# BoxLib-Codes/VARDEN

Hardware: AMD Instinct MI355X
Metric: cells*steps/sec on advance_timestep (higher is better)
Workload: dtype f64; 1 GPU; 3D 256x256x256 single-level variable-density bubble, 1 box(es) of 256^3, MAC+HG projection each step (BASELINE.json configs[1]); parallelism=single GPU, cells=16777216

## Files before the change

### include/varden_amd.h

```cpp
#ifndef VARDEN_AMD_H
#define VARDEN_AMD_H
#include <stddef.h>

#ifdef __cplusplus
extern "C" {
#endif

enum {
  VDN_PERIODIC = -1, VDN_INTERIOR = 0, VDN_INLET = 11, VDN_OUTLET = 12, VDN_SYMMETRY = 13,
  VDN_SLIP_WALL = 14, VDN_NO_SLIP_WALL = 15,
  VDN_REFLECT_ODD = 20, VDN_REFLECT_EVEN = 21, VDN_FOEXTRAP = 22, VDN_EXT_DIR = 23, VDN_HOEXTRAP = 24,
  VDN_BC_PER = -1, VDN_BC_INT = 0, VDN_BC_DIR = 1, VDN_BC_NEU = 2
};

enum { VDN_INITIAL_PROJECTION = 1, VDN_DIVU_ITERS = 2, VDN_PRESSURE_ITERS = 3, VDN_REGULAR_TIMESTEP = 4 };

typedef struct vdn_params {
  int    dm;
  int    nscal;
  int    slope_order;
  int    use_minion;
  int    boussinesq;
  int    stencil_order;
  int    diffusion_type;
// ... 190 lines not shown
        const char *const *names, const vdn_box *pd0, const double *prob_lo, const double *prob_hi,
        double time, const double *dx0, long staging_bytes);
int vdn_fabio_ml_multifab_info (const char *dirname, int *nlev, int *dm, int *ncomp, int nodal[3], int *nboxes, int *rr, double *time);
int vdn_fabio_ml_multifab_boxes(const char *dirname, int lev, vdn_box *boxes, int maxboxes);
int vdn_fabio_ml_multifab_read_d(const char *dirname, int nlev, vdn_multifab *const *mfs, long staging_bytes);
int vdn_checkpoint_write(const char *dirname, int nlev, vdn_multifab *const *state, vdn_multifab *const *pressure,
        const int *rr, double time, double dt, long staging_bytes);
int vdn_checkpoint_info (const char *dirname, int *nlev, double *time, double *dt, int *rr);
int vdn_fabio_ml_multifab_write_plane_d(const char *dirname, int nlev, vdn_multifab *const *mfs, const int *rr,
        const char *const *names, const vdn_box *pd0, const double *prob_lo, const double *prob_hi,
        double time, const double *dx0, long staging_bytes, int ncomp, const int *comps, int nvanish, const int *vanish, double *defect );
int vdn_fabio_ml_multifab_read_plane_d(const char *dirname, int nlev, vdn_multifab *const *mfs, long staging_bytes, int ncomp, const int *comps);
int vdn_checkpoint_write_plane(const char *dirname, int nlev, vdn_multifab *const *state, vdn_multifab *const *pressure,
        const int *rr, double time, double dt, long staging_bytes, int ncomp, const int *comps, int nvanish, const int *vanish, double *defect );
int vdn_make_vorticity_plane(vdn_multifab *vort, int comp, vdn_multifab *u, const double *dx , const vdn_bc_tower *bct);

int  vdn_last_step_timing(double *sec5);
int  vdn_last_solver_stats(int which , int *cycles, double *res0, double *res);
int  vdn_last_bottom_stats(int which , int *calls, int *iters, int *max_iters, int *breakdowns);
int  vdn_last_bottom_form(int which );
int  vdn_last_mac_level_form(void);

int  vdn_k_slope(const vdn_multifab *s, vdn_multifab *slope, int dir, int bccomp, const vdn_bc_tower *bct);
int  vdn_k_velpred(const vdn_multifab *u, vdn_multifab **umac, const vdn_multifab *force,
                   const double *dx, double dt, const vdn_bc_tower *bct);
int  vdn_k_mkflux(const vdn_multifab *s, vdn_multifab **sedge, vdn_multifab **flux,
                  vdn_multifab **umac, const vdn_multifab *force, const vdn_multifab *mac_rhs,
                  const double *dx, double dt, const vdn_bc_tower *bct, int is_vel, const int *is_cons);
int  vdn_k_update(const vdn_multifab *sold, vdn_multifab **umac, vdn_multifab **sedge, vdn_multifab **flux,
                  const vdn_multifab *force, vdn_multifab *snew, const double *dx, double dt,
                  int is_vel, const int *is_cons, const vdn_bc_tower *bct);
int  vdn_k_mkvelforce(vdn_multifab *vel_force, const vdn_multifab *ext_vel_force, const vdn_multifab *s,
                      const vdn_multifab *gp, const vdn_multifab *lapu , double visc_fac,
                      const vdn_bc_tower *bct);
int  vdn_k_mkscalforce(vdn_multifab *scal_force, const vdn_multifab *ext_scal_force,
                       const vdn_multifab *laps , double diff_fac, const vdn_bc_tower *bct);
int  vdn_k_make_at_halftime(vdn_multifab *rhohalf, const vdn_multifab *sold, const vdn_multifab *snew,
                            int in_comp, int out_comp, const vdn_bc_tower *bct);

int  vdn_cc_solve(vdn_multifab *rh, vdn_multifab *phi, vdn_multifab **beta, const double *dx,
                  const int *bc , double rel_eps, double abs_eps, int max_iter,
                  int *cycles, double *res0, double *res);
int  vdn_cc_solve_alpha(vdn_multifab *rh, vdn_multifab *phi, const vdn_multifab *alpha, vdn_multifab **beta, const double *dx,
                        const int *bc , double rel_eps, double abs_eps, int max_iter,
                        int *cycles, double *res0, double *res);
int  vdn_cc_smooth(vdn_multifab *rh, vdn_multifab *phi, vdn_multifab **beta, const double *dx,
// ... 15 lines not shown
```

### varden_amd/advance.py

```python
import ctypes as C

from . import capi
from .boxlib import handle_array
from .capi import check


def _dx(dx):
    flat = [float(v) for lev in dx for v in lev] if hasattr(dx[0], "__len__") else [float(v) for v in dx]
    return (C.c_double * len(flat))(*flat)


def advance_timestep(istep, mla, sold, uold, snew, unew, gp, p, ext_vel_force, ext_scal_force,
                     the_bc_tower, dt, time, dx, press_comp, proj_type):
    lib = capi.load()
    check(lib.vdn_advance_timestep(istep, mla.h, handle_array(sold), handle_array(uold), handle_array(snew),
                                   handle_array(unew), handle_array(gp), handle_array(p),
                                   handle_array(ext_vel_force), handle_array(ext_scal_force), the_bc_tower.h,
                                   float(dt), float(time), _dx(dx), press_comp, proj_type))


def estdt(lev, u, s, gp, ext_vel_force, dx, dtold):
    out = C.c_double()
    check(capi.load().vdn_estdt(lev, u.h, s.h, gp.h, ext_vel_force.h, _dx(dx), float(dtold), C.byref(out)))
    return out.value
# ... 18 lines not shown

def last_solver_stats(which):
    cyc, r0, r = C.c_int(), C.c_double(), C.c_double()
    capi.load().vdn_last_solver_stats(0 if which == "mac" else 1, C.byref(cyc), C.byref(r0), C.byref(r))
    return cyc.value, r0.value, r.value


def last_bottom_stats(which):
    v = [C.c_int() for _ in range(4)]
    check(capi.load().vdn_last_bottom_stats(0 if which == "mac" else 1, *[C.byref(x) for x in v]))
    return dict(calls=v[0].value, iters=v[1].value, max_iters=v[2].value, breakdowns=v[3].value)


def last_bottom_form(which):
    return int(capi.load().vdn_last_bottom_form(0 if which == "mac" else 1))


def _iv(x):
    return (C.c_int * len(x))(*[int(v) for v in x])


def slope(s, slope_mf, dir, bccomp, bct):
    check(capi.load().vdn_k_slope(s.h, slope_mf.h, dir, bccomp, bct.h))


def velpred(u, umac, force, dx, dt, bct):
    check(capi.load().vdn_k_velpred(u.h, handle_array(umac), force.h, _dx(dx), float(dt), bct.h))


def mkflux(s, sedge, flux, umac, force, mac_rhs, dx, dt, bct, is_vel, is_conservative):
    check(capi.load().vdn_k_mkflux(s.h, handle_array(sedge), handle_array(flux), handle_array(umac), force.h, mac_rhs.h,
                                   _dx(dx), float(dt), bct.h, 1 if is_vel else 0, _iv(is_conservative)))


def update(sold, umac, sedge, flux, force, snew, dx, dt, is_vel, is_cons, bct):
    check(capi.load().vdn_k_update(sold.h, handle_array(umac), handle_array(sedge), handle_array(flux), force.h, snew.h,
                                   _dx(dx), float(dt), 1 if is_vel else 0, _iv(is_cons), bct.h))


def mkvelforce(vel_force, ext_vel_force, s, gp, lapu, visc_fac, bct):
    check(capi.load().vdn_k_mkvelforce(vel_force.h, ext_vel_force.h, s.h, gp.h, lapu.h if lapu else None, float(visc_fac), bct.h))


def mkscalforce(scal_force, ext_scal_force, laps, diff_fac, bct):
    check(capi.load().vdn_k_mkscalforce(scal_force.h, ext_scal_force.h, laps.h if laps else None, float(diff_fac), bct.h))

# ... 541 lines not shown
```

### varden_amd/capi.py

```python
import ctypes as C
import os

_HERE = os.path.dirname(os.path.abspath(__file__))
FLAVOUR = "testing" if os.environ.get("VDN_LIB_FLAVOUR") == "testing" else "release"
LIB_PATH = os.path.join(_HERE, "csrc", "libvarden_amd_testing.so" if FLAVOUR == "testing" else "libvarden_amd.so")


class Params(C.Structure):
    _fields_ = [
        ("dm", C.c_int), ("nscal", C.c_int), ("slope_order", C.c_int), ("use_minion", C.c_int),
        ("boussinesq", C.c_int), ("stencil_order", C.c_int), ("diffusion_type", C.c_int),
        ("verbose", C.c_int), ("mg_verbose", C.c_int), ("prob_type", C.c_int),
        ("visc_coef", C.c_double), ("diff_coef", C.c_double), ("cflfac", C.c_double),
        ("max_dt_growth", C.c_double),
        ("u_bc", (C.c_double * 2) * 3), ("v_bc", (C.c_double * 2) * 3), ("w_bc", (C.c_double * 2) * 3),
        ("rho_bc", (C.c_double * 2) * 3), ("trac_bc", (C.c_double * 2) * 3),
        ("mg_nu1", C.c_int), ("mg_nu2", C.c_int), ("mg_nub", C.c_int), ("mg_max_iter", C.c_int),
        ("hg_max_iter", C.c_int), ("hg_nu1", C.c_int), ("hg_nu2", C.c_int), ("hg_nub", C.c_int),
        ("hg_omega", C.c_double), ("mac_rel_eps", C.c_double), ("hg_rel_eps", C.c_double),
        ("abort_on_max_iter", C.c_int), ("hg_fmg", C.c_int), ("mac_fmg", C.c_int), ("hg_omega_pre1", C.c_double), ("hg_omega_pre2", C.c_double),
        ("hg_omega_fac1", C.c_double), ("hg_omega_fac2", C.c_double), ("hg_omega_fac3", C.c_double), ("mg_predict", C.c_int),
        ("mg_bottom_solver", C.c_int), ("hg_bottom_solver", C.c_int), ("max_mg_bottom_nlevels", C.c_int),
        ("mg_bottom_solver_eps", C.c_double), ("hg_bottom_solver_eps", C.c_double),
    ]
# ... 140 lines not shown
    "vdn_particles_count": (C.c_int, [_VP, C.POINTER(C.c_long), C.POINTER(C.c_long)]),
    "vdn_particles_get": (C.c_int, [_VP, _PD, _PI]),
    "vdn_particles_advance": (C.c_int, [_VP, C.c_int, _VP, _PVP, _PVP, _PD, _VP, C.c_double]),
    "vdn_particles_sample": (C.c_int, [_VP, C.c_int, _VP, _PVP, C.c_int, C.c_int, C.c_int, _PD, _VP, _PD, _PI]),
    "vdn_particles_write": (C.c_int, [_VP, C.c_char_p, C.c_double, C.c_int, C.POINTER(C.c_char_p), _PD]),
    "vdn_particles_read": (C.c_int, [C.c_char_p, _PVP, _PD]),
    "vdn_fabio_ml_multifab_write_d": (C.c_int, [C.c_char_p, C.c_int, _PVP, _PI, C.POINTER(C.c_char_p), C.POINTER(Box), _PD, _PD, C.c_double, _PD, C.c_long]),
    "vdn_fabio_ml_multifab_info": (C.c_int, [C.c_char_p, _PI, _PI, _PI, _PI, _PI, _PI, _PD]),
    "vdn_fabio_ml_multifab_boxes": (C.c_int, [C.c_char_p, C.c_int, C.POINTER(Box), C.c_int]),
    "vdn_fabio_ml_multifab_read_d": (C.c_int, [C.c_char_p, C.c_int, _PVP, C.c_long]),
    "vdn_checkpoint_write": (C.c_int, [C.c_char_p, C.c_int, _PVP, _PVP, _PI, C.c_double, C.c_double, C.c_long]),
    "vdn_checkpoint_info": (C.c_int, [C.c_char_p, _PI, _PD, _PD, _PI]),
    "vdn_fabio_ml_multifab_write_plane_d": (C.c_int, [C.c_char_p, C.c_int, _PVP, _PI, C.POINTER(C.c_char_p), C.POINTER(Box), _PD, _PD, C.c_double, _PD, C.c_long,
                                                      C.c_int, _PI, C.c_int, _PI, _PD]),
    "vdn_fabio_ml_multifab_read_plane_d": (C.c_int, [C.c_char_p, C.c_int, _PVP, C.c_long, C.c_int, _PI]),
    "vdn_checkpoint_write_plane": (C.c_int, [C.c_char_p, C.c_int, _PVP, _PVP, _PI, C.c_double, C.c_double, C.c_long, C.c_int, _PI, C.c_int, _PI, _PD]),
    "vdn_make_vorticity_plane": (C.c_int, [_VP, C.c_int, _VP, C.POINTER(C.c_double), _VP]),
    "vdn_last_step_timing": (C.c_int, [_PD]),
    "vdn_last_solver_stats": (C.c_int, [C.c_int, _PI, _PD, _PD]),
    "vdn_last_bottom_stats": (C.c_int, [C.c_int, _PI, _PI, _PI, _PI]),
    "vdn_last_bottom_form": (C.c_int, [C.c_int]),
    "vdn_last_mac_level_form": (C.c_int, []),
    "vdn_k_slope": (C.c_int, [_VP, _VP, C.c_int, C.c_int, _VP]),
    "vdn_k_velpred": (C.c_int, [_VP, _PVP, _VP, _PD, C.c_double, _VP]),
    "vdn_k_mkflux": (C.c_int, [_VP, _PVP, _PVP, _PVP, _VP, _VP, _PD, C.c_double, _VP, C.c_int, _PI]),
    "vdn_k_update": (C.c_int, [_VP, _PVP, _PVP, _PVP, _VP, _VP, _PD, C.c_double, C.c_int, _PI, _VP]),
    "vdn_k_mkvelforce": (C.c_int, [_VP, _VP, _VP, _VP, _VP, C.c_double, _VP]),
    "vdn_k_mkscalforce": (C.c_int, [_VP, _VP, _VP, C.c_double, _VP]),
    "vdn_k_make_at_halftime": (C.c_int, [_VP, _VP, _VP, C.c_int, C.c_int, _VP]),
    "vdn_cc_solve": (C.c_int, [_VP, _VP, _PVP, _PD, _PI, C.c_double, C.c_double, C.c_int, _PI, _PD, _PD]),
    "vdn_cc_solve_alpha": (C.c_int, [_VP, _VP, _VP, _PVP, _PD, _PI, C.c_double, C.c_double, C.c_int, _PI, _PD, _PD]),
    "vdn_cc_smooth": (C.c_int, [_VP, _VP, _PVP, _PD, _PI, C.c_int]),
    "vdn_nd_solve": (C.c_int, [_VP, _VP, _VP, _VP, _PD, _PI, C.c_double, C.c_double, C.c_int, _PI, _PD, _PD]),
    "vdn_bench_cc_smoother": (C.c_int, [_VP, _VP, _PVP, _VP, _PD, _PI, C.c_int, _PD, C.POINTER(C.c_long)]),
    "vdn_bench_cc_smoother_in_solve": (C.c_int, [_VP, _VP, _PVP, _VP, _PD, _PI, C.c_int, C.c_int, _PD, C.POINTER(C.c_long)]),
}

_lib = None


class VardenError(RuntimeError):
    pass


def load():
    global _lib
# ... 19 lines not shown
```

### varden_amd/csrc/advance.hip

```cpp
#include "vdn_dev.h"
#include <chrono>
#include <cmath>

static double wall() { return std::chrono::duration<double>(std::chrono::steady_clock::now().time_since_epoch()).count(); }
static void sync() { HIPCHK(hipStreamSynchronize(ctx().stream)); }


static void restrict_and_fill(int nlev, vdn_multifab **mf, int icomp, int bcomp, int nc, bool same_boundary, const vdn_bc_tower *bct) {
  if (nlev == 1) mf_restrict_and_fill(mf[0], icomp, bcomp, nc, same_boundary, bct);
  else ml_restrict_and_fill(nlev, mf, icomp, bcomp, nc, same_boundary, bct);
}

static void dbg_phase_hash(const char *tag, int nlevs, vdn_multifab **mfs, int per_level = 1, bool whole = false) {
  if (!sw().phase_hash) return;
  HIPCHK(hipStreamSynchronize(ctx().stream));
  unsigned long long h = 1469598103934665603ull;
  for (int n = 0; n < nlevs; n++) for (int q = 0; q < per_level; q++) {
    const vdn_multifab *m = mfs[per_level == 1 ? n : 3 * n + q];
    if (!m) continue;
    std::vector<unsigned long long> buf(m->bytes / 8);
    HIPCHK(hipMemcpy(buf.data(), m->base, m->bytes, hipMemcpyDeviceToHost));
    for (int b = 0; b < m->nfabs(); b++) {
      const FV &f = m->fabs[b]; vdn_box vb = m->vbox[b];
      if (whole) for (int d = 0; d < 3; d++) { vb.lo[d] -= m->ng; vb.hi[d] += m->ng; }
// ... 244 lines not shown
  VDN_TRY
  REQUIRE(mla && mla->nlev <= VDN_MAXLEV, "hgproject: at most %d levels are implemented (nlevel = %d)", VDN_MAXLEV, mla ? mla->nlev : -1);
  arena_reset(); arena_reserve_for(mla);
  do_hgproject(proj_type, mla, unew, uold, rhohalf, p, gp, dx, dt, bct, press_comp - 1);
  arena_reset();
  VDN_CATCH
}
extern "C" int vdn_macproject(vdn_layout *mla, vdn_multifab **umac, vdn_multifab **rho, vdn_multifab **mac_rhs,
                              const double *dx, const vdn_bc_tower *bct, int bc_comp) {
  VDN_TRY
  REQUIRE(mla && mla->nlev <= VDN_MAXLEV, "macproject: at most %d levels are implemented (nlevel = %d)", VDN_MAXLEV, mla ? mla->nlev : -1);
  arena_reset(); arena_reserve_for(mla);
  do_macproject(mla, umac, rho, mac_rhs, dx, bct, bc_comp - 1);
  arena_reset();
  VDN_CATCH
}

#define HOOK_BEGIN(mf) VDN_TRY REQUIRE(ctx().inited, "vdn_init has not been called"); arena_reset(); arena_reserve_for((mf)->la);
#define HOOK_END arena_reset(); VDN_CATCH

extern "C" int vdn_k_slope(const vdn_multifab *s, vdn_multifab *slope, int dir, int bccomp, const vdn_bc_tower *bct) {
  HOOK_BEGIN(s) k_slope(s, slope, dir, bccomp, bct); HOOK_END
}
extern "C" int vdn_k_velpred(const vdn_multifab *u, vdn_multifab **umac, const vdn_multifab *force, const double *dx, double dt,
                             const vdn_bc_tower *bct) {
  HOOK_BEGIN(u)
  k_velpred(u, umac, force, dx, dt, bct);
  for (int d = 0; d < ctx().prm.dm; d++) mf_fill_boundary(umac[d]);
  HOOK_END
}
extern "C" int vdn_k_mkflux(const vdn_multifab *s, vdn_multifab **sedge, vdn_multifab **flux, vdn_multifab **umac,
                            const vdn_multifab *force, const vdn_multifab *mac_rhs, const double *dx, double dt,
                            const vdn_bc_tower *bct, int is_vel, const int *is_cons) {
  HOOK_BEGIN(s) k_mkflux(s, sedge, flux, umac, force, mac_rhs, dx, dt, bct, is_vel != 0, is_cons); HOOK_END
}
extern "C" int vdn_k_update(const vdn_multifab *sold, vdn_multifab **umac, vdn_multifab **sedge, vdn_multifab **flux,
                            const vdn_multifab *force, vdn_multifab *snew, const double *dx, double dt,
                            int is_vel, const int *is_cons, const vdn_bc_tower *bct) {
  HOOK_BEGIN(sold)
  k_update(sold, umac, sedge, flux, force, snew, dx, dt, is_vel != 0, is_cons);
  mf_restrict_and_fill(snew, 0, is_vel ? 0 : bct->dm, snew->nc, false, bct);
  HOOK_END
}
extern "C" int vdn_k_mkvelforce(vdn_multifab *vf, const vdn_multifab *ext, const vdn_multifab *s, const vdn_multifab *gp,
                                const vdn_multifab *lapu, double visc_fac, const vdn_bc_tower *bct) {
  HOOK_BEGIN(vf)
// ... 75 lines not shown
```

### varden_amd/csrc/godunov.hip

```cpp
#include "vdn_dev.h"
#include <algorithm>
#include <type_traits>

struct GArgs {
  int lo[3], hi[3];
  int phys[3][2];
  int adv[3][2][3];
  double dx[3], dt;
  int ncomp, is_vel, use_minion, slope_order;
  int cons[3];
  int outlet2d;
};

template <int D> DEVI double ld(const FV &f, int i, int j, int k, int off, int c = 0) {
  return fv_get(f, i + (D == 0 ? off : 0), j + (D == 1 ? off : 0), k + (D == 2 ? off : 0), c);
}
template <int D> DEVI int coord(int i, int j, int k) { return D == 0 ? i : (D == 1 ? j : k); }
DEVI double sgn1(double x) { return copysign(1.0, x); }

struct Fromm { double cen, lim, flag, fromm; };
DEVI Fromm fromm_of(double sm, double s0, double sp) {
  Fromm f;
  f.cen = 0.5 * (sp - sm);
  double dmin = 2.0 * (s0 - sm), dpls = 2.0 * (sp - s0);
// ... 87 lines not shown
    #pragma unroll
    for (int c = 0; c < NC; c++) {
      w[c][0] = w[c][1]; w[c][1] = w[c][2]; w[c][2] = w[c][3]; w[c][3] = w[c][4]; w[c][4] = SPL(c, k + 2);
      #pragma unroll
      for (int q = 0; q < 4; q++) y[c][q] = SPY(c, k, q);
    }
    #pragma unroll
    for (int c = 0; c < NC; c++) {
      const double s0 = w[c][2];
      const double xm1 = lane_prev(s0), xp1 = lane_next(s0), xm2 = lane_prev(xm1), xp2 = lane_next(xp1);
      if (own_ij) {
        fv_at(sl0, i, j, k, c) = slope_vals(xm2, xm1, s0, xp1, xp2, i, A.lo[0], A.hi[0], SPEC(0, 0, c), SPEC(0, 1, c), A.slope_order);
        fv_at(sl2, i, j, k, c) = slope_vals(w[c][0], w[c][1], s0, w[c][3], w[c][4], k, A.lo[2], A.hi[2], SPEC(2, 0, c), SPEC(2, 1, c), A.slope_order);
        fv_at(sl1, i, j, k, c) = slope_vals(y[c][0], y[c][1], s0, y[c][2], y[c][3], j, A.lo[1], A.hi[1], SPEC(1, 0, c), SPEC(1, 1, c), A.slope_order);
      }
      if (own_ij && vmax && i >= A.lo[0] && i <= A.hi[0] && j >= A.lo[1] && j <= A.hi[1] && k >= A.lo[2] && k <= A.hi[2]) m = fmax(m, fabs(s0));
    }
  }
  #undef SPL
  #undef SPY
  #undef SPEC
  if (vmax) block_atomic_max(vmax, m);
}
static void launch_slopes(const FV &s, const FV sl[3], const GArgs &A, const Range3 &rg, int ncomp, double *vmax, hipStream_t st) {
  if (sw().slopes_march && (ncomp == 2 || ncomp == 3) && s.a0 <= A.lo[0] - 3 && s.a1 <= A.lo[1] - 3 && s.a2 <= A.lo[2] - 3) {
    const int nx = rg.hi[0] - rg.lo[0] + 1, ny = rg.hi[1] - rg.lo[1] + 1, nz = rg.hi[2] - rg.lo[2] + 1;
    const int tiles = ((nx + 59) / 60) * ((ny + 3) / 4);
    int chunks = std::max(1, std::min(nz / 8, (32 * 256 + tiles - 1) / tiles));
    const int klen = (nz + chunks - 1) / chunks;
    const dim3 g((nx + 59) / 60, (ny + 3) / 4, (nz + klen - 1) / klen), blk(64, 4, 1);
    if (ncomp == 3) hipLaunchKernelGGL(kk_slopes_my<3>, g, blk, 0, st, s, sl[0], sl[1], sl[2], A, rg, klen, vmax);
    else hipLaunchKernelGGL(kk_slopes_my<2>, g, blk, 0, st, s, sl[0], sl[1], sl[2], A, rg, klen, vmax);
    return;
  }
  hipLaunchKernelGGL(kk_slopes, grid_for(rg), dim3(64, 4, 1), 0, st, s, sl[0], sl[1], sl[2], A, rg, 7, vmax);
}

DEVI void bc_pair(double &L, double &R, int phys, int side, bool is_vel, bool normal, double ghost, bool quirk) {
  if (phys == VDN_INLET) { L = ghost; R = ghost; }
  else if (phys == VDN_SLIP_WALL) {
    if (is_vel && normal) { L = 0.0; R = 0.0; }
    else if (side == 0) L = R; else R = L;
  } else if (phys == VDN_NO_SLIP_WALL) {
    if (is_vel) { L = 0.0; R = 0.0; }
    else if (side == 0) L = R; else R = L;
  } else if (phys == VDN_OUTLET) {
    if (is_vel && normal) {
      double v;
      if (side == 0) v = fmin(R, 0.0);
      else v = quirk ? fmin(L, 0.0) : fmax(L, 0.0);
      L = v; R = v;
    } else if (side == 0) L = R; else R = L;
  }
}
template <int D> DEVI int face_side(const GArgs &A, int i, int j, int k) {
  const int f = coord<D>(i, j, k);
  return f == A.lo[D] ? 0 : (f == A.hi[D] + 1 ? 1 : -1);
// ... 773 lines not shown
  (void)nc_unused;
  FV f; f.p = p; f.a0 = b.lo[0] - 1; f.a1 = b.lo[1] - 1; f.a2 = b.lo[2] - 1;
  f.n0 = b.hi[0] - b.lo[0] + 3; f.n1 = b.hi[1] - b.lo[1] + 3; f.n2 = b.hi[2] - b.lo[2] + 3;
  f.sc = (long)f.n0 * f.n1 * f.n2;
  return f;
}

void k_slope(const vdn_multifab *s, vdn_multifab *slope, int dir, int bccomp, const vdn_bc_tower *bct) {
  REQUIRE(s->ng >= 3 && slope->ng == 1 && slope->nc >= s->nc, "k_slope: need s.ng>=3, slope.ng==1, slope.nc>=s.nc");
  if (s->nc > 3) {
    for (int c0 = 0; c0 < s->nc; c0 += 3) {
      const int w = std::min(3, s->nc - c0);
      const vdn_multifab sw = comp_window(s, c0, w);
      vdn_multifab lw = comp_window(slope, c0, w);
      k_slope(&sw, &lw, dir, bccomp + c0, bct);
    }
    return;
  }
  for (int i = 0; i < s->nfabs(); i++) {
    GArgs A; fill_gargs(A, s, i, bct, bccomp, s->nc, nullptr, 0.0);
    Range3 r; for (int d = 0; d < 3; d++) { r.lo[d] = A.lo[d] - 1; r.hi[d] = A.hi[d] + 1; }
    hipLaunchKernelGGL(kk_slopes, grid_for(r), dim3(64, 4, 1), 0, ctx().stream, s->fabs[i], slope->fabs[i], slope->fabs[i], slope->fabs[i], A, r, 1 << dir);
  }
}

static bool mkflux_window(const vdn_multifab *s, vdn_multifab **sedge, vdn_multifab **flux, vdn_multifab **umac,
                          const vdn_multifab *force, const vdn_multifab *mac_rhs, const double *dx, double dt,
                          const vdn_bc_tower *bct, bool is_vel, int bccomp, const int *is_cons, const MkUpdate *upd) {
  if (ctx().prm.dm == 2) { k2_mkflux(s, sedge, flux, umac, force, mac_rhs, dx, dt, bct, is_vel, bccomp, is_cons); return false; }
  bool updated = false;
  const int ncomp = s->nc;
  REQUIRE(ncomp <= 3, "mkflux: at most 3 components per window (got %d)", ncomp);
  REQUIRE(s->ng >= 3 && umac[0]->ng >= 1 && force->ng >= 1 && mac_rhs->ng >= 1, "mkflux: ghost widths");
  hipStream_t st = ctx().stream;
  if (use_batched(s) && !sw().godunov_plain) {
    size_t mark = arena_mark();
    const int nb = s->nfabs();
    GodBatch<MkD> B; B.d.resize(nb);
    double *umax = (double *)arena_alloc(sizeof(double) * nb);
    HIPCHK(hipMemsetAsync(umax, 0, sizeof(double) * nb, st));
    std::vector<FBatchD> fd((size_t)nb * ncomp);
    std::vector<int> fstart((size_t)nb * ncomp);
    bool ok = true, inflow = false;
    for (int ib = 0; ib < nb && ok; ib++) {
      MkD &q = B.d[ib];
      fill_gargs(q.A, s, ib, bct, bccomp, ncomp, dx, dt);
// ... 959 lines not shown
```

### varden_amd/csrc/runtime.hip

```cpp
#include "vdn_dev.h"
#include <algorithm>
#include <chrono>
#include <map>
#include <tuple>

static VdnCtx g_ctx;
VdnCtx &ctx() { return g_ctx; }
static thread_local char g_err[1024] = "";

void vdn_set_error(const char *fmt, ...) { va_list ap; va_start(ap, fmt); vsnprintf(g_err, sizeof g_err, fmt, ap); va_end(ap); }
void vdn_fail(const char *fmt, ...) {
  char buf[1024]; va_list ap; va_start(ap, fmt); vsnprintf(buf, sizeof buf, fmt, ap); va_end(ap);
  throw VdnErr(buf);
}

static std::vector<vdn_multifab *> g_temp_mfs;
void arena_reset() {
  dbg_sync(16);
  for (vdn_multifab *m : g_temp_mfs) delete m;
  g_temp_mfs.clear();
  if (sw().arena_poison && g_ctx.arena && g_ctx.arena_peak > 0) HIPCHK(hipMemsetAsync(g_ctx.arena, 0xFF, std::min(g_ctx.arena_peak + (size_t)(64 << 20), g_ctx.arena_bytes), g_ctx.stream));
  g_ctx.arena_off = 0;
  g_ctx.drop_step_caches();
}
// ... 144 lines not shown
  if (done) return;
  done = true;
  for (char **e = environ; e && *e; e++) {
    if (strncmp(*e, "VDN_", 4) != 0 || !strncmp(*e, "VDN_BENCH_", 10) || !strncmp(*e, "VDN_WORKER_", 11)) continue;
    const char *eq = strchr(*e, '=');
    const size_t len = eq ? (size_t)(eq - *e) : strlen(*e);
    bool known = false;
    for (const SwitchInfo &s : switch_table) if (strlen(s.name) == len && !strncmp(s.name, *e, len)) known = true;
    if (!strncmp(*e, "VDN_LIB_FLAVOUR", 15)) continue;
    if (!known) fprintf(stderr, "varden_amd: warning: environment variable %.*s is not a switch of this library (vdn_debug_switches lists them)\n", (int)len, *e);
#ifndef VDN_TESTING_BUILD
    else fprintf(stderr, "varden_amd: note: %.*s is set but this is the release build: launch-form switches are compiled out (libvarden_amd_testing.so reads them)\n", (int)len, *e);
#endif
  }
}
#ifdef VDN_TESTING_BUILD
unsigned nd_last_prolong_levels();
extern "C" unsigned vdn_nd_prolong_fused_levels(void) { return nd_last_prolong_levels(); }
unsigned nd_last_lds_levels();
extern "C" unsigned vdn_nd_lds_levels(void) { return nd_last_lds_levels(); }
int cc_last_tail_form();
int nd_last_tail_form();
extern "C" int vdn_last_tail_form(int which) { return which == 0 ? cc_last_tail_form() : nd_last_tail_form(); }
#endif
extern "C" const char *vdn_debug_switches(void) {
  static std::string out;
#ifndef VDN_TESTING_BUILD
  if (out.empty()) out = "release build: the switches below are compiled out, every launch form is the default one (libvarden_amd_testing.so reads them)\n";
#endif
  if (out.find(std::string(switch_table[0].name) + " ") == std::string::npos) for (const SwitchInfo &s : switch_table) { const char *v = switch_raw(s); out += s.name; out += v ? std::string(" = ") + v : std::string(" (unset)"); out += ": "; out += s.doc; out += "\n"; }
  return out.c_str();
}

bool g_capturing_now();
__global__ void k_publish(double *host_view, const double *dev, int n, unsigned long long seq) {
  if ((int)threadIdx.x < n) host_view[threadIdx.x] = dev[threadIdx.x];
  __syncthreads();
  if (threadIdx.x == 0) { __threadfence_system(); *reinterpret_cast<volatile unsigned long long *>(host_view + 64) = seq; }
}
const double *read_scalars(const double *dev, int n) {
  VdnCtx &c = g_ctx;
  REQUIRE(n >= 1 && n <= 64, "read_scalars: 1..64 values");
  static unsigned long long seq = 0;
  const bool poll = sw().poll >= 0 ? sw().poll != 0 : c.nranks == 1;
  ++seq;
  dbg_sync(8);
// ... 750 lines not shown
```

### varden_amd/csrc/vdn_internal.h

```cpp
#pragma once
#define VDN_MAXLEV 4
#include <hip/hip_runtime.h>
#include <string>
#include <vector>
#include <map>
#include <cstdio>
#include <cstdarg>
#include <cstring>
#include <cstdlib>
#include <stdexcept>
#include <cmath>
#include "../../include/varden_amd.h"
#include "vdn_switches.h"
#include "mg_plan.h"

struct FV {
  double *p;
  int a0, a1, a2;
  int n0, n1, n2;
  long sc;
};
struct BoxP {
  int lo[3], hi[3];
  int phys[3][2];
// ... 207 lines not shown
    }
    std::sort(out.begin(), out.end()); out.erase(std::unique(out.begin(), out.end()), out.end());
    return out;
  }
};
BoxP make_boxp(const vdn_multifab *mf, int i, const vdn_bc_tower *bct);
void mf_setval(vdn_multifab *mf, double val, int comp, int nc, bool all);
void mf_fill_boundary(vdn_multifab *mf, bool faces_only = false);
void mf_physbc(vdn_multifab *mf, int scomp, int bccomp, int nc, const vdn_bc_tower *bct, bool same_boundary = false);
void mf_copy(vdn_multifab *dst, int dcomp, const vdn_multifab *src, int scomp, int nc, int ng);
double mf_norm_inf(const vdn_multifab *mf, int comp, int nc);
double mf_norm_inf_grown(const vdn_multifab *mf, int comp, int nc, int grow);
double mf_max_ratio3(vdn_multifab *const *a, vdn_multifab *const *b);
void mf_restrict_and_fill(vdn_multifab *mf, int icomp, int bcomp, int nc, bool same_boundary, const vdn_bc_tower *bct);

bool god_per_box(const vdn_multifab *s);
void k_velpred(const vdn_multifab *u, vdn_multifab **umac, const vdn_multifab *force, const double *dx, double dt,
               const vdn_bc_tower *bct);
struct MkUpdate { vdn_multifab *snew = nullptr; int fmode = 0; const vdn_multifab *ext = nullptr, *gp = nullptr, *rho = nullptr; double lapu0 = 0.0; };
bool k_mkflux(const vdn_multifab *s, vdn_multifab **sedge, vdn_multifab **flux, vdn_multifab **umac,
              const vdn_multifab *force, const vdn_multifab *mac_rhs, const double *dx, double dt,
              const vdn_bc_tower *bct, bool is_vel, const int *is_cons, const MkUpdate *upd = nullptr);
void k_slope(const vdn_multifab *s, vdn_multifab *slope, int dir, int bccomp, const vdn_bc_tower *bct);
void k_update_velforce(const vdn_multifab *uold, vdn_multifab **umac, vdn_multifab **uedge, const vdn_multifab *ext, const vdn_multifab *s,
                       const vdn_multifab *gp, const vdn_multifab *lapu, double visc_fac, vdn_multifab *unew, const double *dx, double dt);
void k_update(const vdn_multifab *sold, vdn_multifab **umac, vdn_multifab **sedge, vdn_multifab **flux,
              const vdn_multifab *force, vdn_multifab *snew, const double *dx, double dt, bool is_vel, const int *is_cons);
void k_mkvelforce(vdn_multifab *vf, const vdn_multifab *ext, const vdn_multifab *s, const vdn_multifab *gp,
                  const vdn_multifab *lapu, double visc_fac);
void k_mkscalforce(vdn_multifab *sf, const vdn_multifab *ext, const vdn_multifab *laps, double diff_fac);
void k_make_at_halftime(vdn_multifab *rhohalf, const vdn_multifab *sold, const vdn_multifab *snew, int in_comp, int out_comp);
void k_estdt_max(const vdn_multifab *u, const vdn_multifab *s, const vdn_multifab *gp, const vdn_multifab *ext, double out6[6]);
void do_macproject(vdn_layout *mla, vdn_multifab **umac, vdn_multifab **rho, vdn_multifab **mac_rhs, const double *dx,
                   const vdn_bc_tower *bct, int bc_comp0);
struct CcFast { vdn_multifab **um = nullptr; const vdn_multifab *mac_rhs = nullptr, *rho = nullptr; std::vector<FV> phi_view; };
struct MgRequest {
  const double *dx = nullptr;
  const int (*bc)[2] = nullptr;
  double rel_eps = 0.0, abs_eps = -1.0;
  int max_iter = 0;
  int cycles = 0;
  double res0 = 0.0, res = 0.0;
};
struct MgLevelRequest : MgRequest {
  int fixed_cycles = 0;
  vdn_multifab *add_to = nullptr;
// ... 73 lines not shown
```

### varden_amd/csrc/vdn_switches.h

```cpp
#pragma once
#include <algorithm>
#include <cstddef>
#include <cstdlib>
#include <cstring>

#define VDN_SWITCHES(X) \
  X(testing, "VDN_TESTING", STR, nullptr, "1: allows VDN_RCCL_LIB (the test transport of tests/fake_rccl); nothing else") \
  X(rccl_lib, "VDN_RCCL_LIB", STR, nullptr, "path of a library that stands in for librccl -- honoured only with VDN_TESTING=1 and the test double's handshake") \
  X(force_packed, "VDN_FORCE_PACKED", LIVE, 0, "1: box-to-box copies of one rank go through the packed per-peer buffers (device memcpy for send/recv); 2: through a 1-rank RCCL communicator (one-GPU rehearsal of the N > 1 transport)") \
  X(arena_poison, "VDN_ARENA_POISON", SET, false, "1: every byte handed back to the arena is overwritten with NaNs (a read of an entry nobody wrote fails the next solve)") \
  X(arena_chunk, "VDN_ARENA_CHUNK_MB", MB, (size_t)1024 << 20, "size of the physical chunks mapped into the arena's address range (default 1024)") \
  X(field_chunk, "VDN_FIELD_CHUNK_MB", MB, (size_t)64 << 20, "size of the pooled physical chunks behind the state fields (default 64)") \
  X(field_vmm, "VDN_FIELD_VMM", ON, true, "0: every state field is one hipMalloc block (rounds 1-5) instead of pooled chunks mapped into its own address range") \
  X(mlcc_trace, "VDN_MLCC_TRACE", SET, false, "1: the composite cell-centred solve prints its residual at every FAC iteration (stderr)") \
  X(keep_off, "VDN_KEEP_OFF", INT, 0, "mask of kept-descriptor families rebuilt at every call: 1 generic sets, 2 create_umac_grown, 4 composite cell-centred solve, 8 nodal prolongation") \
  X(sync_points, "VDN_SYNC_POINTS", INT, 0, "mask of points that synchronise the device (race hunting): 1 after every batched launch, 2 after every staged upload, 4 after every exchange, 8 before a scalar read-back, 16 at arena_reset, 32 after launch_cells") \
  X(phase_hash, "VDN_PHASE_HASH", SET, false, "1: advance_timestep prints a checksum of its fields at every phase boundary (stderr)") \
  X(no_roctx, "VDN_NO_ROCTX", PRESENT, false, "do not bind the roctx library (no bl_prof ranges)") \
  X(poll, "VDN_POLL", INT, -1, "scalar read-back: 1 spin on the pinned sequence number, 0 hipStreamSynchronize; default: spin on one rank, synchronise on several") \
  X(no_graphs, "VDN_NO_GRAPHS", PRESENT, false, "launch every multigrid cycle eagerly instead of replaying its hipGraph") \
  X(no_slope_cache, "VDN_NO_SLOPE_CACHE", PRESENT, false, "velocity mkflux recomputes the slopes of uold that velpred computed in the same step") \
  X(no_force_reuse, "VDN_NO_FORCE_REUSE", SET, false, "1: every forcing term is computed where the reference computes it (advance_premac AND velocity_advance, ...)") \
  X(slopes_march, "VDN_SLOPES_MARCH", ON, true, "0: the per-cell slopes kernel instead of the k-marching one") \
  X(godunov_batch, "VDN_GODUNOV_BATCH", SET, false, "1: the descriptor (box-batched) Godunov kernels also on a level of one box") \
  X(godunov_plain, "VDN_GODUNOV_PLAIN", PRESENT, false, "the face-centred one-thread-per-cell Godunov kernels of round 1 (the fused marches' bit-for-bit reference, and their fallback where they refuse the field layouts)") \
  X(god_segw, "VDN_GOD_SEGW", ON, true, "0: the box-batched fused Godunov marches use full-width (64 x 8) tiles for every box") \
  X(god_p2, "VDN_GOD_P2", ON, true, "0: the fused marches divide by dx also where every dx is a power of two (default there: scale by 1/dx, the same doubles)") \
  X(fused_kchunks, "VDN_FUSED_KCHUNKS", MIN1, 0, "k-chunks of the fused marches (default: the count that fills the last round of workgroups best)") \
  X(god_update, "VDN_GOD_UPDATE", ON, true, "0: update_3d as its own pass instead of inside the fused mkflux march") \
  X(gsrb_pair, "VDN_GSRB_PAIR", ON, true, "0: one cell per thread in the colour passes / residuals of wide levels instead of the 2 x 2 pair form") \
  X(mac_split, "VDN_MAC_SPLIT", ON, true, "0: the finest level of macproject's one-level solve stays interleaved (kk_cc_gsrb_rho_pair) instead of stored by colour (kk_cc_gsrb_rho_split)") \
  X(mac_split_min, "VDN_MAC_SPLIT_MIN", INT, 1<<23, "fewest cells (of this rank's boxes together) of a level stored by colour (default 2^23)") \
  X(nd_rev, "VDN_ND_REV", ON, true, "0: every march of a nodal level walks its tiles in the same order (default: consecutive marches alternate)") \
  X(mac_slab, "VDN_MAC_SLAB", INT, -1, "planes per slab of the time-skewed schedule of the split level's passes (cc_split_run; default: ~200 MB of pass traffic, at most half the level); 0: whole-level launches") \
  X(mac_umax, "VDN_MAC_UMAX", ON, true, "0: max |umac| by its own pass (kk_macmax) instead of inside macproject's velocity update (kk_mkumac_rho_max)") \
  X(mac_kflip, "VDN_MAC_KFLIP", ON, true, "0: both colour passes of a sweep walk the planes upwards (default: the second colour downwards; paired and split passes of the cell-centred multigrid)") \
  X(cc_halo_faces, "VDN_CC_HALO_FACES", ON, true, "0: the cell-centred multigrid exchanges the whole ghost shell instead of the faces only") \
  X(overlap, "VDN_OVERLAP", INT, -1, "halo exchange of multigrid passes next to interior work: 1 always, 0 never, default: when a plan has a remote peer and the box is large") \
  X(mg_agglom, "VDN_MG_AGGLOM", INT, 0, "box width below which a multi-box multigrid level is gathered into one box (default: 64 across ranks, 128 where every box is this rank's)") \
  X(mg_restrict_fused, "VDN_MG_RESTRICT_FUSED", ON, true, "0: cell-centred residual and restriction as two passes") \
  X(mg_tailcycle, "VDN_MG_TAILCYCLE", ON, true, "0: the smallest levels launch by launch instead of one single-workgroup cycle") \
  X(mg_prolong_fused, "VDN_MG_PROLONG_FUSED", ON, true, "0: cell-centred prolongation as its own pass instead of inside the first post-smoothing colour pass") \
  X(mg_lds, "VDN_MG_LDS", ON, true, "0: the 16^3..64^3-cell levels of both multigrids (cell-centred and nodal) launch by launch instead of the LDS-tiled down / up kernels") \
  X(mac_stored_beta, "VDN_MAC_STORED_BETA", SET, false, "1: the finest MAC level reads stored face coefficients instead of recomputing them from rho") \
  X(mac_fast, "VDN_MAC_FAST", ON, true, "0: macproject with its rh / phi / beta multifabs as the reference has them") \
  X(hg_fast, "VDN_HG_FAST", ON, true, "0: hgproject with its rh / phi / coeffs multifabs as the reference has them") \
// ... 53 lines not shown
```

Measured before the change: 698.8 million cells*steps/s.

## Add pair-form k-marching slopes kernel with LDS y-neighbours and double2 lanes

Adds kk_slopes_pr, a slopes kernel that marches in k. Each lane handles two x-cells loaded as a double2, and the y-neighbours are shared through a double-buffered LDS tile with halo rows. A planner picks the tile widths and k-chunking. It becomes the default (switch value 2) wherever the field layouts meet the alignment and ghost-cell checks, otherwise it falls back to the old march. The aim is fewer redundant global loads and wider memory transactions for slope computation, at the cost of one LDS barrier per plane and idle edge lanes in each tile.

```diff
diff --git a/include/varden_amd.h b/include/varden_amd.h
--- a/include/varden_amd.h
+++ b/include/varden_amd.h
@@ -236,6 +236,7 @@
 int  vdn_last_mac_level_form(void);
 
 int  vdn_k_slope(const vdn_multifab *s, vdn_multifab *slope, int dir, int bccomp, const vdn_bc_tower *bct);
+int  vdn_k_slopes_march(const vdn_multifab *s, vdn_multifab *sl0, vdn_multifab *sl1, vdn_multifab *sl2, int bccomp, const vdn_bc_tower *bct, double *vmax);
 int  vdn_k_velpred(const vdn_multifab *u, vdn_multifab **umac, const vdn_multifab *force,
                    const double *dx, double dt, const vdn_bc_tower *bct);
 int  vdn_k_mkflux(const vdn_multifab *s, vdn_multifab **sedge, vdn_multifab **flux,
diff --git a/varden_amd/advance.py b/varden_amd/advance.py
--- a/varden_amd/advance.py
+++ b/varden_amd/advance.py
@@ -64,6 +64,12 @@
 
 def slope(s, slope_mf, dir, bccomp, bct):
     check(capi.load().vdn_k_slope(s.h, slope_mf.h, dir, bccomp, bct.h))
+
+
+def slopes_march(s, sl, bccomp, bct, want_max=False):
+    m = C.c_double(0.0)
+    check(capi.load().vdn_k_slopes_march(s.h, sl[0].h, sl[1].h, sl[2].h, bccomp, bct.h, C.byref(m) if want_max else None))
+    return m.value if want_max else None
 
 
 def velpred(u, umac, force, dx, dt, bct):
diff --git a/varden_amd/capi.py b/varden_amd/capi.py
--- a/varden_amd/capi.py
+++ b/varden_amd/capi.py
@@ -186,6 +186,7 @@
     "vdn_last_bottom_form": (C.c_int, [C.c_int]),
     "vdn_last_mac_level_form": (C.c_int, []),
     "vdn_k_slope": (C.c_int, [_VP, _VP, C.c_int, C.c_int, _VP]),
+    "vdn_k_slopes_march": (C.c_int, [_VP, _VP, _VP, _VP, C.c_int, _VP, C.POINTER(C.c_double)]),
     "vdn_k_velpred": (C.c_int, [_VP, _PVP, _VP, _PD, C.c_double, _VP]),
     "vdn_k_mkflux": (C.c_int, [_VP, _PVP, _PVP, _PVP, _VP, _VP, _PD, C.c_double, _VP, C.c_int, _PI]),
     "vdn_k_update": (C.c_int, [_VP, _PVP, _PVP, _PVP, _VP, _VP, _PD, C.c_double, C.c_int, _PI, _VP]),
diff --git a/varden_amd/csrc/advance.hip b/varden_amd/csrc/advance.hip
--- a/varden_amd/csrc/advance.hip
+++ b/varden_amd/csrc/advance.hip
@@ -290,6 +290,9 @@
 extern "C" int vdn_k_slope(const vdn_multifab *s, vdn_multifab *slope, int dir, int bccomp, const vdn_bc_tower *bct) {
   HOOK_BEGIN(s) k_slope(s, slope, dir, bccomp, bct); HOOK_END
 }
+extern "C" int vdn_k_slopes_march(const vdn_multifab *s, vdn_multifab *sl0, vdn_multifab *sl1, vdn_multifab *sl2, int bccomp, const vdn_bc_tower *bct, double *vmax) {
+  HOOK_BEGIN(s) k_slopes_march(s, sl0, sl1, sl2, bccomp, bct, vmax); HOOK_END
+}
 extern "C" int vdn_k_velpred(const vdn_multifab *u, vdn_multifab **umac, const vdn_multifab *force, const double *dx, double dt,
                              const vdn_bc_tower *bct) {
   HOOK_BEGIN(u)
diff --git a/varden_amd/csrc/godunov.hip b/varden_amd/csrc/godunov.hip
--- a/varden_amd/csrc/godunov.hip
+++ b/varden_amd/csrc/godunov.hip
@@ -1,4 +1,5 @@
 #include "vdn_dev.h"
+#include "slopes_plan.h"
 #include <algorithm>
 #include <type_traits>
 
@@ -133,9 +134,93 @@
   #undef SPEC
   if (vmax) block_atomic_max(vmax, m);
 }
+template <int NC> __global__ void __launch_bounds__(64 * SLP_WAVES) kk_slopes_pr(FV s, FV sl0, FV sl1, FV sl2, GArgs A, Range3 r, SlopesPlan P, double *vmax) {
+  __shared__ double2 sm[2][(SLP_WAVES + 4) * 64];
+  const int tid = threadIdx.x, c = blockIdx.z;
+  int lw, pair0, by, pl, rr, hrow, hslot;
+  slopes_tile(P, (int)blockIdx.x, lw, pair0, by);
+  const bool own_l = slopes_lane(lw, tid, pl, rr), hal = slopes_halo(lw, tid, hrow, hslot);
+  const int W = 1 << lw, j0 = r.lo[1] + by * (SLP_WAVES * (64 >> lw));
+  const int i_ = r.lo[0] + 2 * (pair0 + pl - 1), j_ = j0 + rr;
+  const bool own = own_l && i_ <= r.hi[0] && j_ <= r.hi[1];
+  const int ic = min(max(i_, A.lo[0] - 3), A.hi[0] + 2), jc = min(max(j_, A.lo[1] - 3), A.hi[1] + 3), jh = min(max(j0 + hrow, A.lo[1] - 3), A.hi[1] + 3);
+  const int k0 = r.lo[2] + (int)blockIdx.y * P.klen, k1 = min(k0 + P.klen - 1, r.hi[2]);
+  const long sp = (long)s.n0 * s.n1, slp = (long)sl0.n0 * sl0.n1;
+  const double *pw = s.p + s.sc * c + fv_idx(s, ic, jc, s.a2), *ph = s.p + s.sc * c + fv_idx(s, ic, hal ? jh : jc, s.a2);
+  const long so = fv_idx(sl0, own ? i_ : r.lo[0], own ? j_ : r.lo[1], sl0.a2) + sl0.sc * c;
+  #define SPL(p, kk) (*(const double2 *)((p) + (long)(min(max((kk), A.lo[2] - 3), A.hi[2] + 3) - s.a2) * sp))
+  #define SPEC(d, sd) (A.adv[d][sd][c] == VDN_EXT_DIR || A.adv[d][sd][c] == VDN_HOEXTRAP)
+  const bool xl = SPEC(0, 0), xh = SPEC(0, 1), yl = SPEC(1, 0), yh = SPEC(1, 1), zl = SPEC(2, 0), zh = SPEC(2, 1);
+  const int o = A.slope_order;
+  double2 w[5], nx, hv;
+  w[0] = make_double2(0.0, 0.0);
+  #pragma unroll
+  for (int q = 1; q < 5; q++) w[q] = SPL(pw, k0 - 3 + q);
+  nx = SPL(pw, k0 + 2);
+  hv = SPL(ph, k0);
+  const int o0 = (rr + 2) * W + pl, oh = hslot * W + pl;
+  double m = 0.0;
+  int b = 0;
+  for (int k = k0; k <= k1; k++, b ^= 1) {
+    w[0] = w[1]; w[1] = w[2]; w[2] = w[3]; w[3] = w[4]; w[4] = nx;
+    sm[b][o0] = w[2];
+    if (hal) sm[b][oh] = hv;
+    nx = SPL(pw, k + 3);
+    if (hal) hv = SPL(ph, k + 1);
+    __syncthreads();
+    const double2 s0 = w[2];
+    const double2 y0 = sm[b][o0 - 2 * W], y1 = sm[b][o0 - W], y2 = sm[b][o0 + W], y3 = sm[b][o0 + 2 * W];
+    const double pa = lane_prev(s0.x), pb = lane_prev(s0.y), na = lane_next(s0.x), nb = lane_next(s0.y);
+    if (own) {
+      const int i = i_, j = j_;
+      double2 d0, d1, d2;
+      d0.x = slope_vals(pa, pb, s0.x, s0.y, na, i, A.lo[0], A.hi[0], xl, xh, o);
+      d0.y = slope_vals(pb, s0.x, s0.y, na, nb, i + 1, A.lo[0], A.hi[0], xl, xh, o);
+      d2.x = slope_vals(w[0].x, w[1].x, s0.x, w[3].x, w[4].x, k, A.lo[2], A.hi[2], zl, zh, o);
+      d2.y = slope_vals(w[0].y, w[1].y, s0.y, w[3].y, w[4].y, k, A.lo[2], A.hi[2], zl, zh, o);
+      d1.x = slope_vals(y0.x, y1.x, s0.x, y2.x, y3.x, j, A.lo[1], A.hi[1], yl, yh, o);
+      d1.y = slope_vals(y0.y, y1.y, s0.y, y2.y, y3.y, j, A.lo[1], A.hi[1], yl, yh, o);
+      const long oc = so + (long)(k - sl0.a2) * slp;
+      *(double2 *)(sl0.p + oc) = d0; *(double2 *)(sl2.p + oc) = d2; *(double2 *)(sl1.p + oc) = d1;
+      if (vmax && j >= A.lo[1] && j <= A.hi[1] && k >= A.lo[2] && k <= A.hi[2]) {
+        if (i >= A.lo[0] && i <= A.hi[0]) m = fmax(m, fabs(s0.x));
+        if (i + 1 >= A.lo[0] && i + 1 <= A.hi[0]) m = fmax(m, fabs(s0.y));
+      }
+    }
+  }
+  #undef SPL
+  #undef SPEC
+  if (vmax) block_atomic_max(vmax, m);
+}
+static int g_slopes_form = 0;
+int slopes_last_form() { return g_slopes_form; }
+static bool slopes_pair_fits(const FV &s, const FV sl[3], const GArgs &A, const Range3 &rg) {
+  for (int d = 0; d < 3; d++) {
+    if (rg.lo[d] != A.lo[d] - 1 || rg.hi[d] != A.hi[d] + 1) return false;
+    const int a = d == 0 ? s.a0 : d == 1 ? s.a1 : s.a2, n = d == 0 ? s.n0 : d == 1 ? s.n1 : s.n2;
+    const int b = d == 0 ? sl[0].a0 : d == 1 ? sl[0].a1 : sl[0].a2, nb = d == 0 ? sl[0].n0 : d == 1 ? sl[0].n1 : sl[0].n2;
+    if (a > A.lo[d] - 3 || a + n - 1 < A.hi[d] + 3 || b > rg.lo[d] || b + nb - 1 < rg.hi[d]) return false;
+  }
+  const SlopesLayout Ls = { (long)rg.lo[0] - s.a0, s.n0, s.sc, (uintptr_t)s.p };
+  for (int d = 0; d < 3; d++) {
+    if (sl[d].a0 != sl[0].a0 || sl[d].a1 != sl[0].a1 || sl[d].a2 != sl[0].a2 || sl[d].n0 != sl[0].n0 || sl[d].n1 != sl[0].n1 || sl[d].sc != sl[0].sc) return false;
+    const SlopesLayout Ll = { (long)rg.lo[0] - sl[d].a0, sl[d].n0, sl[d].sc, (uintptr_t)sl[d].p };
+    if (!slopes_pair_ok(rg.hi[0] - rg.lo[0] + 1, rg.lo[0] - (A.lo[0] - 3), A.hi[0] + 3 - rg.hi[0], Ls, Ll)) return false;
+  }
+  return true;
+}
 static void launch_slopes(const FV &s, const FV sl[3], const GArgs &A, const Range3 &rg, int ncomp, double *vmax, hipStream_t st) {
   if (sw().slopes_march && (ncomp == 2 || ncomp == 3) && s.a0 <= A.lo[0] - 3 && s.a1 <= A.lo[1] - 3 && s.a2 <= A.lo[2] - 3) {
     const int nx = rg.hi[0] - rg.lo[0] + 1, ny = rg.hi[1] - rg.lo[1] + 1, nz = rg.hi[2] - rg.lo[2] + 1;
+    if (sw().slopes_march >= 2 && slopes_pair_fits(s, sl, A, rg)) {
+      const SlopesPlan P = slopes_plan(nx, ny, nz);
+      const dim3 g(P.tiles, P.chunks, ncomp), blk(64 * SLP_WAVES, 1, 1);
+      if (ncomp == 3) hipLaunchKernelGGL(kk_slopes_pr<3>, g, blk, 0, st, s, sl[0], sl[1], sl[2], A, rg, P, vmax);
+      else hipLaunchKernelGGL(kk_slopes_pr<2>, g, blk, 0, st, s, sl[0], sl[1], sl[2], A, rg, P, vmax);
+      g_slopes_form = 2;
+      return;
+    }
+    g_slopes_form = 1;
     const int tiles = ((nx + 59) / 60) * ((ny + 3) / 4);
     int chunks = std::max(1, std::min(nz / 8, (32 * 256 + tiles - 1) / tiles));
     const int klen = (nz + chunks - 1) / chunks;
@@ -144,6 +229,7 @@
     else hipLaunchKernelGGL(kk_slopes_my<2>, g, blk, 0, st, s, sl[0], sl[1], sl[2], A, rg, klen, vmax);
     return;
   }
+  g_slopes_form = 0;
   hipLaunchKernelGGL(kk_slopes, grid_for(rg), dim3(64, 4, 1), 0, st, s, sl[0], sl[1], sl[2], A, rg, 7, vmax);
 }
 
@@ -963,6 +1049,21 @@
     Range3 r; for (int d = 0; d < 3; d++) { r.lo[d] = A.lo[d] - 1; r.hi[d] = A.hi[d] + 1; }
     hipLaunchKernelGGL(kk_slopes, grid_for(r), dim3(64, 4, 1), 0, ctx().stream, s->fabs[i], slope->fabs[i], slope->fabs[i], slope->fabs[i], A, r, 1 << dir);
   }
+}
+
+void k_slopes_march(const vdn_multifab *s, vdn_multifab *sl0, vdn_multifab *sl1, vdn_multifab *sl2, int bccomp, const vdn_bc_tower *bct, double *vmax) {
+  REQUIRE((s->nc == 2 || s->nc == 3) && s->ng >= 3, "k_slopes_march: s needs 2 or 3 components and 3 ghost cells");
+  REQUIRE(sl0->ng == 1 && sl1->ng == 1 && sl2->ng == 1 && sl0->nc == s->nc && sl1->nc == s->nc && sl2->nc == s->nc, "k_slopes_march: the slope multifabs need 1 ghost cell and the components of s");
+  hipStream_t st = ctx().stream;
+  double *dmax = nullptr;
+  if (vmax) { dmax = (double *)arena_alloc(256); HIPCHK(hipMemsetAsync(dmax, 0, sizeof(double), st)); }
+  for (int ib = 0; ib < s->nfabs(); ib++) {
+    GArgs A; fill_gargs(A, s, ib, bct, bccomp, s->nc, nullptr, 0.0);
+    Range3 rg; for (int d = 0; d < 3; d++) { rg.lo[d] = A.lo[d] - 1; rg.hi[d] = A.hi[d] + 1; }
+    const FV sl[3] = { sl0->fabs[ib], sl1->fabs[ib], sl2->fabs[ib] };
+    launch_slopes(s->fabs[ib], sl, A, rg, s->nc, dmax, st);
+  }
+  if (vmax) *vmax = read_scalar1(dmax);
 }
 
 static bool mkflux_window(const vdn_multifab *s, vdn_multifab **sedge, vdn_multifab **flux, vdn_multifab **umac,
diff --git a/varden_amd/csrc/runtime.hip b/varden_amd/csrc/runtime.hip
--- a/varden_amd/csrc/runtime.hip
+++ b/varden_amd/csrc/runtime.hip
@@ -190,6 +190,8 @@
 int cc_last_tail_form();
 int nd_last_tail_form();
 extern "C" int vdn_last_tail_form(int which) { return which == 0 ? cc_last_tail_form() : nd_last_tail_form(); }
+int slopes_last_form();
+extern "C" int vdn_last_slopes_form(void) { return slopes_last_form(); }
 #endif
 extern "C" const char *vdn_debug_switches(void) {
   static std::string out;
diff --git a/varden_amd/csrc/slopes_plan.h b/varden_amd/csrc/slopes_plan.h
--- /dev/null
+++ b/varden_amd/csrc/slopes_plan.h
@@ -0,0 +1,64 @@
+#pragma once
+#include <cstdint>
+#if defined(__HIPCC__)
+#define SLP_FN __host__ __device__ inline
+#else
+#define SLP_FN inline
+#endif
+
+#define SLP_WAVES 8
+#define SLP_WG_TARGET 1024
+#define SLP_LDS_BUDGET 40960
+
+struct SlopesPlan {
+  int gxm, gy;
+  int lwr, gyr;
+  int tiles;
+  int klen, chunks;
+};
+struct SlopesLayout { long off0, n0, sc; uintptr_t base; };
+
+SLP_FN bool slopes_layout_ok(const SlopesLayout &L) { return (L.off0 & 1) == 0 && L.off0 >= 0 && (L.n0 & 1) == 0 && (L.sc & 1) == 0 && (L.base & 15) == 0; }
+SLP_FN bool slopes_pair_ok(int nx, int lo_gap, int hi_gap, const SlopesLayout &s, const SlopesLayout &sl) {
+  return nx >= 2 && (nx & 1) == 0 && lo_gap == 2 && hi_gap == 2 && s.off0 >= 2 && s.off0 + nx + 2 <= s.n0 && sl.off0 + nx <= sl.n0 && slopes_layout_ok(s) && slopes_layout_ok(sl);
+}
+SLP_FN int slopes_lds_bytes() { return 2 * (SLP_WAVES + 4) * 64 * 16; }
+
+SLP_FN SlopesPlan slopes_plan(int nx, int ny, int nz, int wg_target = SLP_WG_TARGET) {
+  SlopesPlan P;
+  const int npairs = nx / 2;
+  P.gxm = npairs / 62;
+  int rem = npairs - 62 * P.gxm;
+  P.lwr = 6; P.gyr = 0;
+  if (rem > 30) { P.gxm++; rem = 0; }
+  P.gy = P.gxm ? (ny + SLP_WAVES - 1) / SLP_WAVES : 0;
+  if (rem > 0) {
+    P.lwr = 2; while ((1 << P.lwr) - 2 < rem) P.lwr++;
+    const int rows = SLP_WAVES * (64 >> P.lwr);
+    P.gyr = (ny + rows - 1) / rows;
+  }
+  P.tiles = P.gxm * P.gy + P.gyr;
+  int chunks = (wg_target + P.tiles - 1) / P.tiles;
+  if (chunks > nz / 8) chunks = nz / 8;
+  if (chunks < 1) chunks = 1;
+  P.klen = (nz + chunks - 1) / chunks;
+  P.chunks = (nz + P.klen - 1) / P.klen;
+  return P;
+}
+SLP_FN void slopes_tile(const SlopesPlan &P, int t, int &lw, int &pair0, int &by) {
+  const int nmain = P.gxm * P.gy;
+  if (t < nmain) { lw = 6; pair0 = (t % P.gxm) * 62; by = t / P.gxm; }
+  else { lw = P.lwr; pair0 = P.gxm * 62; by = t - nmain; }
+}
+SLP_FN bool slopes_lane(int lw, int tid, int &pl, int &rr) {
+  const int W = 1 << lw;
+  pl = tid & (W - 1); rr = tid >> lw;
+  return pl >= 1 && pl <= W - 2;
+}
+SLP_FN bool slopes_halo(int lw, int tid, int &drow, int &slot) {
+  const int W = 1 << lw, rows = SLP_WAVES * (64 >> lw), h = tid >> lw;
+  if (tid >= 4 * W) { drow = slot = 0; return false; }
+  drow = h < 2 ? h - 2 : rows + h - 2;
+  slot = h < 2 ? h : rows + h;
+  return true;
+}
diff --git a/varden_amd/csrc/vdn_internal.h b/varden_amd/csrc/vdn_internal.h
--- a/varden_amd/csrc/vdn_internal.h
+++ b/varden_amd/csrc/vdn_internal.h
@@ -253,6 +253,7 @@
               const vdn_multifab *force, const vdn_multifab *mac_rhs, const double *dx, double dt,
               const vdn_bc_tower *bct, bool is_vel, const int *is_cons, const MkUpdate *upd = nullptr);
 void k_slope(const vdn_multifab *s, vdn_multifab *slope, int dir, int bccomp, const vdn_bc_tower *bct);
+void k_slopes_march(const vdn_multifab *s, vdn_multifab *sl0, vdn_multifab *sl1, vdn_multifab *sl2, int bccomp, const vdn_bc_tower *bct, double *vmax);
 void k_update_velforce(const vdn_multifab *uold, vdn_multifab **umac, vdn_multifab **uedge, const vdn_multifab *ext, const vdn_multifab *s,
                        const vdn_multifab *gp, const vdn_multifab *lapu, double visc_fac, vdn_multifab *unew, const double *dx, double dt);
 void k_update(const vdn_multifab *sold, vdn_multifab **umac, vdn_multifab **sedge, vdn_multifab **flux,
diff --git a/varden_amd/csrc/vdn_switches.h b/varden_amd/csrc/vdn_switches.h
--- a/varden_amd/csrc/vdn_switches.h
+++ b/varden_amd/csrc/vdn_switches.h
@@ -21,7 +21,7 @@
   X(no_graphs, "VDN_NO_GRAPHS", PRESENT, false, "launch every multigrid cycle eagerly instead of replaying its hipGraph") \
   X(no_slope_cache, "VDN_NO_SLOPE_CACHE", PRESENT, false, "velocity mkflux recomputes the slopes of uold that velpred computed in the same step") \
   X(no_force_reuse, "VDN_NO_FORCE_REUSE", SET, false, "1: every forcing term is computed where the reference computes it (advance_premac AND velocity_advance, ...)") \
-  X(slopes_march, "VDN_SLOPES_MARCH", ON, true, "0: the per-cell slopes kernel instead of the k-marching one") \
+  X(slopes_march, "VDN_SLOPES_MARCH", INT, 2, "0: the per-cell slopes kernel instead of the k-marching one; 1: the march with one cell per lane and its y-neighbours from memory (kk_slopes_my); default 2: its pair form (kk_slopes_pr) wherever the layouts take it") \
   X(godunov_batch, "VDN_GODUNOV_BATCH", SET, false, "1: the descriptor (box-batched) Godunov kernels also on a level of one box") \
   X(godunov_plain, "VDN_GODUNOV_PLAIN", PRESENT, false, "the face-centred one-thread-per-cell Godunov kernels of round 1 (the fused marches' bit-for-bit reference, and their fallback where they refuse the field layouts)") \
   X(god_segw, "VDN_GOD_SEGW", ON, true, "0: the box-batched fused Godunov marches use full-width (64 x 8) tiles for every box") \
```

Result: faster. 706.8 million cells*steps/s, median of 6 (+1.1%).
